# cocowy1/PPMStereo

Measured on AMD Instinct MI355X. Metric: disparity-px/s, higher is better.
Workload: dtype bf16

## Files before the change

### ppmstereo_amd/csrc/loop_ops.hip

```cpp
#include "common.h"

constexpr int DW_PX = 2;
template <int K>
__global__ __launch_bounds__(256) void dwconv_gelu_kernel(ppms_sp x, ppms_sp y, const float* __restrict__ w, const float* __restrict__ b,
                                                          int H, int W, int64_t rows, int groups) {
    __shared__ __attribute__((aligned(16))) float wl[K * K * 64];
    const int C = groups * 8;
    for (int i = threadIdx.x; i < K * K * C; i += 256) {
        const int c = i % C, tap = i / C;
        wl[tap * C + c] = w[c * K * K + tap];
    }
    __syncthreads();
    const int rpr = (W + DW_PX - 1) / DW_PX;
    const int64_t idx = (int64_t)blockIdx.x * 256 + threadIdx.x;
    if (idx >= rows * rpr * groups) return;
    const int c0 = (int)(idx % groups) * 8;
    const int64_t run = idx / groups;
    const int px0 = (int)(run % rpr) * DW_PX;
    const int64_t row = run / rpr;
    const int py = (int)(row % H);
    const int64_t pix0 = row * W + px0;
    const bf16_t* xh = (const bf16_t*)x.hi + c0;
    const bf16_t* xl = (const bf16_t*)x.lo + c0;
    float acc[DW_PX][8], x0[DW_PX][8];
    {
        const f32x4 b0 = *(const f32x4*)(b + c0), b1 = *(const f32x4*)(b + c0 + 4);
#pragma unroll
        for (int p = 0; p < DW_PX; ++p)
#pragma unroll
            for (int j = 0; j < 8; ++j) {
                acc[p][j] = j < 4 ? b0[j & 3] : b1[j & 3];
                x0[p][j] = 0.0f;
            }
    }
    constexpr int R = K / 2, NW = DW_PX + K - 1;
#pragma unroll
    for (int ky = 0; ky < K; ++ky) {
        const int yy = py + ky - R;
        if ((unsigned)yy >= (unsigned)H) continue;
        float win[NW][8];
#pragma unroll
        for (int i = 0; i < NW; ++i) {
            const int xx = px0 - R + i;
            bf16x8 h8 = {0, 0, 0, 0, 0, 0, 0, 0}, l8 = {0, 0, 0, 0, 0, 0, 0, 0};
            if ((unsigned)xx < (unsigned)W) {
                const int64_t q = pix0 + (int64_t)(ky - R) * W + (i - R);
                h8 = *(const bf16x8*)(xh + q * x.ld);
                l8 = *(const bf16x8*)(xl + q * x.ld);
            }
#pragma unroll
            for (int j = 0; j < 8; ++j) win[i][j] = join_bf16(h8[j], l8[j]);
        }
        if (ky == R) {
#pragma unroll
            for (int p = 0; p < DW_PX; ++p)
#pragma unroll
                for (int j = 0; j < 8; ++j) x0[p][j] = win[p + R][j];
        }
#pragma unroll
        for (int kx = 0; kx < K; ++kx) {
            const f32x4 w0 = *(const f32x4*)(wl + (ky * K + kx) * C + c0), w1 = *(const f32x4*)(wl + (ky * K + kx) * C + c0 + 4);
#pragma unroll
            for (int p = 0; p < DW_PX; ++p)
#pragma unroll
                for (int j = 0; j < 8; ++j) acc[p][j] += (j < 4 ? w0[j & 3] : w1[j & 3]) * win[p + kx][j];
        }
    }
#pragma unroll
    for (int p = 0; p < DW_PX; ++p) {
        if (px0 + p >= W) break;
        bf16x8 oh, ol;
#pragma unroll
        for (int j = 0; j < 8; ++j) {
            bf16_t hi, lo;
            split_bf16(gelu_erf(x0[p][j] + acc[p][j]), hi, lo);
            oh[j] = hi;
            ol[j] = lo;
        }
        *(bf16x8*)((bf16_t*)y.hi + (pix0 + p) * y.ld + c0) = oh;
        *(bf16x8*)((bf16_t*)y.lo + (pix0 + p) * y.ld + c0) = ol;
    }
}

extern "C" int ppms_dwconv_gelu(ppms_sp x, ppms_sp y, const float* w, const float* b, int k, int BT, int H, int W, void* stream) {
    PPMS_REQUIRE(k == 1 || k == 7, "dwconv_gelu: k=%d (only 1 and 7)", k);
    PPMS_REQUIRE(x.hi && x.lo && y.hi && y.lo && x.c == y.c && x.c > 0 && x.c <= 64 && x.c % 8 == 0 && x.ld % 8 == 0 && y.ld % 8 == 0,
                 "dwconv_gelu: views must have c <= 64 and c, ld multiples of 8");
    PPMS_REQUIRE((((uintptr_t)x.hi | (uintptr_t)x.lo | (uintptr_t)y.hi | (uintptr_t)y.lo) & 15) == 0,
                 "dwconv_gelu: the planes of x and y must be 16-byte aligned (a view starts at a multiple of 8 channels)");
    PPMS_REQUIRE(w != nullptr && b != nullptr && ((uintptr_t)b & 15) == 0, "dwconv_gelu: w and a 16-byte aligned bias expected");
    PPMS_REQUIRE(BT > 0 && H > 0 && W > 0, "dwconv_gelu: bad shape BT=%d H=%d W=%d", BT, H, W);
    const int64_t rows = (int64_t)BT * H;
    const int groups = x.c / 8;
    const dim3 grid(ceil_div(rows * ((W + DW_PX - 1) / DW_PX) * groups, 256));
    if (k == 1)
        hipLaunchKernelGGL(dwconv_gelu_kernel<1>, grid, dim3(256), 0, (hipStream_t)stream, x, y, w, b, H, W, rows, groups);
    else
        hipLaunchKernelGGL(dwconv_gelu_kernel<7>, grid, dim3(256), 0, (hipStream_t)stream, x, y, w, b, H, W, rows, groups);
    return ppms_check_launch("dwconv_gelu");
}

__global__ __launch_bounds__(256) void flow_patch7_kernel(const float* __restrict__ flow, ppms_sp patch, int H, int W, int64_t P) {
    const int64_t idx = (int64_t)blockIdx.x * 256 + threadIdx.x;
    if (idx >= P * 128) return;
    const int k = (int)(idx & 127);
    const int64_t pix = idx >> 7;
    float v = 0.0f;
    if (k < 98) {
        const int tap = k >> 1, c = k & 1;
        const int ky = tap / 7, kx = tap - ky * 7;
        const int px = (int)(pix % W), py = (int)((pix / W) % H);
        const int xx = px + kx - 3, yy = py + ky - 3;
        if ((unsigned)xx < (unsigned)W && (unsigned)yy < (unsigned)H) v = flow[(pix + (int64_t)(ky - 3) * W + (kx - 3)) * 2 + c];
    }
    bf16_t hi, lo;
    split_bf16(v, hi, lo);
    ((bf16_t*)patch.hi)[pix * patch.ld + k] = hi;
    ((bf16_t*)patch.lo)[pix * patch.ld + k] = lo;
}

extern "C" int ppms_flow_patch7(const float* flow_nhwc, ppms_sp patch, int BT, int H, int W, void* stream) {
    PPMS_REQUIRE(flow_nhwc && patch.hi && patch.lo && patch.ld >= 128, "flow_patch7: bad arguments");
    const int64_t P = (int64_t)BT * H * W;
    hipLaunchKernelGGL(flow_patch7_kernel, dim3(ceil_div(P * 128, 256)), dim3(256), 0, (hipStream_t)stream, flow_nhwc, patch, H, W, P);
    return ppms_check_launch("flow_patch7");
}

__global__ __launch_bounds__(256) void unc_tail_kernel(ppms_sp x, const float* __restrict__ w, float bias, float* __restrict__ unc,
                                                       float* __restrict__ partial, int HW, int nblk) {
    __shared__ float red[16];
    const int frame = blockIdx.y, blk = blockIdx.x;
    const int sub = threadIdx.x & 15, grp = threadIdx.x >> 4;
    float wv[8];
#pragma unroll
    for (int j = 0; j < 8; ++j) wv[j] = w[sub * 8 + j];
    bf16x8 h8[16], l8[16];
#pragma unroll
    for (int it = 0; it < 16; ++it) {
        const int pin = blk * 256 + it * 16 + grp;
        const int64_t pix = (int64_t)frame * HW + (pin < HW ? pin : HW - 1);
        h8[it] = gld<bf16x8>((const bf16_t*)x.hi + pix * x.ld + sub * 8);
        l8[it] = gld<bf16x8>((const bf16_t*)x.lo + pix * x.ld + sub * 8);
    }
    float local = 0.0f;
#pragma unroll
    for (int it = 0; it < 16; ++it) {
        const int pin = blk * 256 + it * 16 + grp;
        float s = 0.0f;
#pragma unroll
        for (int j = 0; j < 8; ++j) s += wv[j] * join_bf16(h8[it][j], l8[it][j]);
        s += __shfl_xor(s, 1);
        s += __shfl_xor(s, 2);
        s += __shfl_xor(s, 4);
        s += __shfl_xor(s, 8);
        if (pin < HW && sub == 0) {
            const float u = sigmoid_f(s + bias);
            unc[(int64_t)frame * HW + pin] = u;
            local += u;
        }
    }
    if (sub == 0) red[grp] = local;
    __syncthreads();
    if (threadIdx.x == 0) {
        float t = 0.0f;
        for (int i = 0; i < 16; ++i) t += red[i];
        partial[frame * nblk + blk] = t;
    }
}

extern "C" int ppms_unc_tail(ppms_sp x, const float* w, float bias, float* unc, float* partial, int BT, int HW, void* stream) {
    PPMS_REQUIRE(x.hi && x.lo && x.c == 128 && x.ld % 8 == 0, "unc_tail: expects a 128-channel SP view");
    const int nblk = ceil_div(HW, 256);
    hipLaunchKernelGGL(unc_tail_kernel, dim3(nblk, BT), dim3(256), 0, (hipStream_t)stream, x, w, bias, unc, partial, HW, nblk);
    return ppms_check_launch("unc_tail");
}

__global__ __launch_bounds__(256) void tap_gather_sum_kernel(const float* __restrict__ y, int y_ld, const float* __restrict__ bias,
                                                             float* __restrict__ out, int out_ld, float* __restrict__ accum, int accum_ld, int cout,
                                                             int kt, int kh, int kw, int T, int H, int W, int t_halo, int64_t total) {
    const int64_t idx = (int64_t)blockIdx.x * 256 + threadIdx.x;
    if (idx >= total) return;
    const int c = (int)(idx % cout);
    const int64_t pix = idx / cout;
    const int x = (int)(pix % W), yy = (int)((pix / W) % H), t = (int)(pix / ((int64_t)W * H));
    float acc = bias ? bias[c] : 0.0f;
    int tap = 0;
    for (int kz = 0; kz < kt; ++kz)
        for (int ky = 0; ky < kh; ++ky)
            for (int kx = 0; kx < kw; ++kx, ++tap) {
                const int tt = t + kz - kt / 2, y2 = yy + ky - kh / 2, x2 = x + kx - kw / 2;
                if ((unsigned)(tt + t_halo) < (unsigned)(T + 2 * t_halo) && (unsigned)y2 < (unsigned)H && (unsigned)x2 < (unsigned)W)
                    acc += y[(((int64_t)tt * H + y2) * W + x2) * y_ld + tap * cout + c];
            }
    out[pix * out_ld + c] = acc;
    if (accum != nullptr) accum[pix * accum_ld + c] += acc;
}
__global__ __launch_bounds__(256) void tap_gather_sum333_kernel(const float* __restrict__ y, int y_ld, const float* __restrict__ bias,
                                                                float* __restrict__ out, int out_ld, float* __restrict__ accum, int accum_ld, int cout,
                                                                int T, int H, int W, int t_halo, int64_t total) {
    const int64_t idx = (int64_t)blockIdx.x * 256 + threadIdx.x;
    if (idx >= total) return;
    const int c = (int)(idx % cout);
    const int64_t pix = idx / cout;
    const int x = (int)(pix % W), yy = (int)((pix / W) % H), t = (int)(pix / ((int64_t)W * H));
    float v[27];
#pragma unroll
    for (int tap = 0; tap < 27; ++tap) {
        const int kz = tap / 9, ky = (tap / 3) % 3, kx = tap % 3;
        const int tt = t + kz - 1, y2 = yy + ky - 1, x2 = x + kx - 1;
        const bool ok = (unsigned)(tt + t_halo) < (unsigned)(T + 2 * t_halo) && (unsigned)y2 < (unsigned)H && (unsigned)x2 < (unsigned)W;
        v[tap] = ok ? y[(((int64_t)tt * H + y2) * W + x2) * y_ld + tap * cout + c] : 0.0f;
    }
    float acc = bias ? bias[c] : 0.0f;
#pragma unroll
    for (int tap = 0; tap < 27; ++tap) {
        const int kz = tap / 9, ky = (tap / 3) % 3, kx = tap % 3;
        const int tt = t + kz - 1, y2 = yy + ky - 1, x2 = x + kx - 1;
        const bool ok = (unsigned)(tt + t_halo) < (unsigned)(T + 2 * t_halo) && (unsigned)y2 < (unsigned)H && (unsigned)x2 < (unsigned)W;
        if (ok) acc += v[tap];
    }
    out[pix * out_ld + c] = acc;
    if (accum != nullptr) accum[pix * accum_ld + c] += acc;
}
extern "C" int ppms_tap_gather_sum(const float* y, int y_ld, const float* bias, float* out, int out_ld, float* accum, int accum_ld, int cout, int kt,
                                   int kh, int kw, int T, int H, int W, int t_halo, void* stream) {
    PPMS_REQUIRE(y && out && cout > 0 && kt * kh * kw * cout <= y_ld && out_ld >= cout && t_halo >= 0, "tap_gather_sum: bad arguments");
    PPMS_REQUIRE(accum == nullptr || accum_ld >= cout, "tap_gather_sum: accum_ld=%d < cout=%d", accum_ld, cout);
    const int64_t total = (int64_t)T * H * W * cout;
    if (kt == 3 && kh == 3 && kw == 3)
        hipLaunchKernelGGL(tap_gather_sum333_kernel, dim3(ceil_div(total, 256)), dim3(256), 0, (hipStream_t)stream, y, y_ld, bias, out, out_ld, accum,
                           accum_ld, cout, T, H, W, t_halo, total);
    else
        hipLaunchKernelGGL(tap_gather_sum_kernel, dim3(ceil_div(total, 256)), dim3(256), 0, (hipStream_t)stream, y, y_ld, bias, out, out_ld, accum, accum_ld,
                           cout, kt, kh, kw, T, H, W, t_halo, total);
    return ppms_check_launch("tap_gather_sum");
}

__global__ __launch_bounds__(256) void flow_add_kernel(float* __restrict__ flow, const float* __restrict__ dflow, int dflow_ld, int64_t P) {
    const int64_t idx = (int64_t)blockIdx.x * 256 + threadIdx.x;
    if (idx >= P * 2) return;
    flow[idx] += dflow[(idx >> 1) * dflow_ld + (idx & 1)];
}
extern "C" int ppms_flow_add(float* flow_nhwc, const float* dflow, int dflow_ld, int64_t pixels, void* stream) {
    PPMS_REQUIRE(flow_nhwc && dflow && dflow_ld >= 2, "flow_add: bad arguments");
    hipLaunchKernelGGL(flow_add_kernel, dim3(ceil_div(pixels * 2, 256)), dim3(256), 0, (hipStream_t)stream, flow_nhwc, dflow, dflow_ld, pixels);
    return ppms_check_launch("flow_add");
}

__global__ __launch_bounds__(256) void convex_upsample_kernel(const float* __restrict__ flow, const float* __restrict__ mask, int mask_ld,
                                                              float* __restrict__ out, int H, int W, int64_t P) {
    const int64_t idx = (int64_t)blockIdx.x * 256 + threadIdx.x;
    if (idx >= P * 16) return;
    const int sub = (int)(idx & 15);
    const int64_t pix = idx >> 4;
    const int x = (int)(pix % W), y = (int)((pix / W) % H);
    const int64_t frame = pix / ((int64_t)H * W);
    const float* m = mask + pix * mask_ld + sub;
    float mv[9], mx = -INFINITY;
#pragma unroll
    for (int k = 0; k < 9; ++k) {
        mv[k] = m[16 * k];
        mx = fmaxf(mx, mv[k]);
    }
    float den = 0.0f;
#pragma unroll
    for (int k = 0; k < 9; ++k) {
        mv[k] = expf(mv[k] - mx);
        den += mv[k];
    }
    float o0 = 0.0f, o1 = 0.0f;
#pragma unroll
    for (int k = 0; k < 9; ++k) {
        const int yy = y + k / 3 - 1, xx = x + k % 3 - 1;
        if ((unsigned)yy < (unsigned)H && (unsigned)xx < (unsigned)W) {
            const int64_t q = pix + (int64_t)(k / 3 - 1) * W + (k % 3 - 1);
            const float wgt = mv[k] / den;
            o0 += wgt * (4.0f * flow[q * 2]);
            o1 += wgt * (4.0f * flow[q * 2 + 1]);
        }
    }
    const int i = sub >> 2, j = sub & 3;
    const int64_t OW = 4 * (int64_t)W, OHW = 16 * (int64_t)H * W;
    const int64_t o = (frame * 2) * OHW + (int64_t)(4 * y + i) * OW + 4 * x + j;
    out[o] = o0;
    out[o + OHW] = o1;
}
extern "C" int ppms_convex_upsample(const float* flow_nhwc, const float* mask, int mask_ld, float* out, int BT, int H, int W, void* stream) {
    PPMS_REQUIRE(flow_nhwc && mask && out && mask_ld >= 144, "convex_upsample: bad arguments");
    const int64_t P = (int64_t)BT * H * W;
    hipLaunchKernelGGL(convex_upsample_kernel, dim3(ceil_div(P * 16, 256)), dim3(256), 0, (hipStream_t)stream, flow_nhwc, mask, mask_ld,
                       out, H, W, P);
    return ppms_check_launch("convex_upsample");
}

__global__ __launch_bounds__(256) void convex_upsample3d_kernel(const float* __restrict__ flow, const float* __restrict__ mask, int mask_ld,
                                                                float* __restrict__ out, int T, int H, int W, int t_halo, int64_t P) {
    const int64_t idx = (int64_t)blockIdx.x * 256 + threadIdx.x;
    if (idx >= P * 16) return;
    const int sub = (int)(idx & 15);
    const int64_t pix = idx >> 4;
    const int x = (int)(pix % W), y = (int)((pix / W) % H);
    const int64_t frame = pix / ((int64_t)W * H);
    const float* mp = mask + pix * mask_ld + sub;
    float mv[27];
    float mx = mp[0];
#pragma unroll
    for (int k = 0; k < 27; ++k) {
        mv[k] = mp[16 * k];
        mx = fmaxf(mx, mv[k]);
    }
    float den = 0.0f;
#pragma unroll
    for (int k = 0; k < 27; ++k) {
        mv[k] = expf(mv[k] - mx);
        den += mv[k];
    }
    float o0 = 0.0f, o1 = 0.0f;
#pragma unroll
    for (int k = 0; k < 27; ++k) {
        const int dt = k / 9 - 1, dy = (k / 3) % 3 - 1, dx = k % 3 - 1;
        const int tt = (int)frame + dt, yy = y + dy, xx = x + dx;
        if ((unsigned)(tt + t_halo) < (unsigned)(T + 2 * t_halo) && (unsigned)yy < (unsigned)H && (unsigned)xx < (unsigned)W) {
            const int64_t q = pix + ((int64_t)dt * H + dy) * W + dx;
            const float wgt = mv[k] / den;
            o0 += wgt * (4.0f * flow[q * 2]);
            o1 += wgt * (4.0f * flow[q * 2 + 1]);
        }
    }
    const int i = sub >> 2, j = sub & 3;
    const int64_t OW = 4 * (int64_t)W, OHW = 16 * (int64_t)H * W;
    const int64_t o = (frame * 2) * OHW + (int64_t)(4 * y + i) * OW + 4 * x + j;
    out[o] = o0;
    out[o + OHW] = o1;
}
extern "C" int ppms_convex_upsample_3d(const float* flow_nhwc, const float* mask, int mask_ld, float* out, int T, int H, int W, int t_halo, void* stream) {
    PPMS_REQUIRE(flow_nhwc && mask && out && mask_ld >= 432 && T > 0 && H > 0 && W > 0 && t_halo >= 0, "convex_upsample_3d: bad arguments");
    const int64_t P = (int64_t)T * H * W;
    hipLaunchKernelGGL(convex_upsample3d_kernel, dim3(ceil_div(P * 16, 256)), dim3(256), 0, (hipStream_t)stream, flow_nhwc, mask, mask_ld,
                       out, T, H, W, t_halo, P);
    return ppms_check_launch("convex_upsample_3d");
}
```

Measured before the change: 23.59 million.

## Software-pipeline depthwise conv row loads and adapt per-thread tile to grid size

Rewrites the depthwise 7x7 conv+GELU kernel so input rows are prefetched several rows ahead into registers. Out-of-bounds taps are clamped rather than branched on, so loads stay unconditional. The kernel also overlaps the weight staging into shared memory with the first row loads, uses 32-bit offsets when the tensor fits, and joins hi/lo bf16 pairs with byte-permute ops. The launcher picks a smaller pixel/channel tile per thread when the grid would otherwise be too small, to keep the GPU occupied. The risk is higher register pressure from prefetch buffers and extra template instantiations.

```diff
diff --git a/ppmstereo_amd/csrc/loop_ops.hip b/ppmstereo_amd/csrc/loop_ops.hip
--- a/ppmstereo_amd/csrc/loop_ops.hip
+++ b/ppmstereo_amd/csrc/loop_ops.hip
@@ -1,85 +1,147 @@
 #include "common.h"
 
-constexpr int DW_PX = 2;
-template <int K>
+constexpr int dw_ahead(int NW, int CH) { return 176 / (NW * CH) < 1 ? 1 : 176 / (NW * CH); }
+constexpr int DW_MIN_THREADS = 65536;
+template <int PX, int CH> __device__ __forceinline__ void dw_pin(float (&a)[PX][CH]) {
+#pragma unroll
+    for (int p = 0; p < PX; ++p)
+#pragma unroll
+        for (int j = 0; j < CH; ++j) asm volatile("" : "+v"(a[p][j])::"memory");
+}
+template <int K, int PX, int CH, class OFS>
 __global__ __launch_bounds__(256) void dwconv_gelu_kernel(ppms_sp x, ppms_sp y, const float* __restrict__ w, const float* __restrict__ b,
                                                           int H, int W, int64_t rows, int groups) {
-    __shared__ __attribute__((aligned(16))) float wl[K * K * 64];
-    const int C = groups * 8;
-    for (int i = threadIdx.x; i < K * K * C; i += 256) {
-        const int c = i % C, tap = i / C;
-        wl[tap * C + c] = w[c * K * K + tap];
-    }
+    typedef bf16_t bfv __attribute__((ext_vector_type(CH)));
+    typedef float fv __attribute__((ext_vector_type(CH)));
+    constexpr int NT = 256;
+    __shared__ __attribute__((aligned(32))) float wl[K * K * 64];
+    constexpr int R = K / 2, NW = PX + K - 1, D = K < dw_ahead(NW, CH) ? K : dw_ahead(NW, CH);
+    const int C = groups * CH;
+    const int rpr = (W + PX - 1) / PX;
+    const OFS total = (OFS)rows * (OFS)rpr * (OFS)groups;
+    const OFS gid = (OFS)blockIdx.x * NT + threadIdx.x;
+    const bool live = gid < total;
+    const OFS idx = live ? gid : total - 1;
+    const OFS run = idx / (OFS)groups;
+    const int c0 = (int)(idx - run * (OFS)groups) * CH;
+    const OFS row = run / (OFS)rpr;
+    const int px0 = (int)(run - row * (OFS)rpr) * PX;
+    const int py = (int)(row % (OFS)H);
+    const int64_t pix0 = (int64_t)row * W + px0;
+    const char* xh = (const char*)x.hi;
+    const char* xl = (const char*)x.lo;
+    const OFS ldb = (OFS)x.ld * 2;
+    OFS col[NW];
+    bool cok[NW];
+#pragma unroll
+    for (int i = 0; i < NW; ++i) {
+        const int xx = px0 - R + i;
+        cok[i] = (unsigned)xx < (unsigned)W;
+        col[i] = (OFS)(xx < 0 ? 0 : (xx >= W ? W - 1 : xx)) * ldb + (OFS)(c0 * 2);
+    }
+    bfv rh[K][NW], rl[K][NW];
+    auto load_row = [&](int ky) __attribute__((always_inline)) {
+        const int yy = py + ky - R;
+        const OFS ro = (OFS)((row - py + (yy < 0 ? 0 : (yy >= H ? H - 1 : yy))) * W) * ldb;
+#pragma unroll
+        for (int i = 0; i < NW; ++i) {
+            rh[ky][i] = gld<bfv>(xh + (ro + col[i]));
+            rl[ky][i] = gld<bfv>(xl + (ro + col[i]));
+        }
+    };
+    float acc[PX][CH], x0[PX][CH];
+#pragma unroll
+    for (int j = 0; j < CH; ++j) acc[0][j] = gld<float>(b + c0 + j);
+#pragma unroll
+    for (int ky = 0; ky < D; ++ky) load_row(ky);
+#pragma unroll 4
+    for (int i = threadIdx.x; i < K * K * C; i += NT) {
+        const int c = i / (K * K), tap = i - c * (K * K);
+        wl[tap * C + c] = w[i];
+    }
+#pragma unroll
+    for (int p = 0; p < PX; ++p)
+#pragma unroll
+        for (int j = 0; j < CH; ++j) {
+            acc[p][j] = acc[0][j];
+            x0[p][j] = 0.0f;
+        }
     __syncthreads();
-    const int rpr = (W + DW_PX - 1) / DW_PX;
-    const int64_t idx = (int64_t)blockIdx.x * 256 + threadIdx.x;
-    if (idx >= rows * rpr * groups) return;
-    const int c0 = (int)(idx % groups) * 8;
-    const int64_t run = idx / groups;
-    const int px0 = (int)(run % rpr) * DW_PX;
-    const int64_t row = run / rpr;
-    const int py = (int)(row % H);
-    const int64_t pix0 = row * W + px0;
-    const bf16_t* xh = (const bf16_t*)x.hi + c0;
-    const bf16_t* xl = (const bf16_t*)x.lo + c0;
-    float acc[DW_PX][8], x0[DW_PX][8];
-    {
-        const f32x4 b0 = *(const f32x4*)(b + c0), b1 = *(const f32x4*)(b + c0 + 4);
-#pragma unroll
-        for (int p = 0; p < DW_PX; ++p)
-#pragma unroll
-            for (int j = 0; j < 8; ++j) {
-                acc[p][j] = j < 4 ? b0[j & 3] : b1[j & 3];
-                x0[p][j] = 0.0f;
+#pragma unroll
+    for (int ky = 0; ky < K; ++ky) {
+        const bool rok = K == 1 || (unsigned)(py + ky - R) < (unsigned)H;
+        float keep[PX][CH];
+#pragma unroll
+        for (int p = 0; p < PX; ++p)
+#pragma unroll
+            for (int j = 0; j < CH; ++j) keep[p][j] = acc[p][j];
+#pragma unroll
+        for (int i = 0; i < NW; ++i) {
+            unsigned hd[CH / 2], lw[CH / 2];
+            __builtin_memcpy(hd, &rh[ky][i], CH * 2);
+            __builtin_memcpy(lw, &rl[ky][i], CH * 2);
+            const unsigned m_odd = cok[i] ? 0xffff0000u : 0u, s_even = cok[i] ? 0x01000c0cu : 0x0c0c0c0cu;
+            float v[CH];
+#pragma unroll
+            for (int q = 0; q < CH / 2; ++q) {
+                v[2 * q] = __builtin_bit_cast(float, __builtin_amdgcn_perm(0u, hd[q], s_even)) + __builtin_bit_cast(float, __builtin_amdgcn_perm(0u, lw[q], s_even));
+                v[2 * q + 1] = __builtin_bit_cast(float, hd[q] & m_odd) + __builtin_bit_cast(float, lw[q] & m_odd);
             }
-    }
-    constexpr int R = K / 2, NW = DW_PX + K - 1;
-#pragma unroll
-    for (int ky = 0; ky < K; ++ky) {
-        const int yy = py + ky - R;
-        if ((unsigned)yy >= (unsigned)H) continue;
-        float win[NW][8];
-#pragma unroll
-        for (int i = 0; i < NW; ++i) {
-            const int xx = px0 - R + i;
-            bf16x8 h8 = {0, 0, 0, 0, 0, 0, 0, 0}, l8 = {0, 0, 0, 0, 0, 0, 0, 0};
-            if ((unsigned)xx < (unsigned)W) {
-                const int64_t q = pix0 + (int64_t)(ky - R) * W + (i - R);
-                h8 = *(const bf16x8*)(xh + q * x.ld);
-                l8 = *(const bf16x8*)(xl + q * x.ld);
+            if (ky == R && i >= R && i < R + PX) {
+#pragma unroll
+                for (int j = 0; j < CH; ++j) x0[i - R][j] = v[j];
             }
 #pragma unroll
-            for (int j = 0; j < 8; ++j) win[i][j] = join_bf16(h8[j], l8[j]);
-        }
-        if (ky == R) {
-#pragma unroll
-            for (int p = 0; p < DW_PX; ++p)
-#pragma unroll
-                for (int j = 0; j < 8; ++j) x0[p][j] = win[p + R][j];
-        }
-#pragma unroll
-        for (int kx = 0; kx < K; ++kx) {
-            const f32x4 w0 = *(const f32x4*)(wl + (ky * K + kx) * C + c0), w1 = *(const f32x4*)(wl + (ky * K + kx) * C + c0 + 4);
-#pragma unroll
-            for (int p = 0; p < DW_PX; ++p)
-#pragma unroll
-                for (int j = 0; j < 8; ++j) acc[p][j] += (j < 4 ? w0[j & 3] : w1[j & 3]) * win[p + kx][j];
-        }
-    }
-#pragma unroll
-    for (int p = 0; p < DW_PX; ++p) {
-        if (px0 + p >= W) break;
-        bf16x8 oh, ol;
-#pragma unroll
-        for (int j = 0; j < 8; ++j) {
+            for (int p = 0; p < PX; ++p) {
+                const int kx = i - p;
+                if (kx < 0 || kx >= K) continue;
+                const fv wv = *(const fv*)(wl + (ky * K + kx) * C + c0);
+#pragma unroll
+                for (int j = 0; j < CH; ++j) acc[p][j] += wv[j] * v[j];
+            }
+        }
+#pragma unroll
+        for (int p = 0; p < PX; ++p)
+#pragma unroll
+            for (int j = 0; j < CH; ++j) acc[p][j] = rok ? acc[p][j] : keep[p][j];
+        dw_pin(acc);
+        if (ky + D < K) load_row(ky + D);
+    }
+#pragma unroll
+    for (int p = 0; p < PX; ++p) {
+        if (!live || px0 + p >= W) break;
+        bfv oh, ol;
+#pragma unroll
+        for (int j = 0; j < CH; ++j) {
             bf16_t hi, lo;
             split_bf16(gelu_erf(x0[p][j] + acc[p][j]), hi, lo);
             oh[j] = hi;
             ol[j] = lo;
         }
-        *(bf16x8*)((bf16_t*)y.hi + (pix0 + p) * y.ld + c0) = oh;
-        *(bf16x8*)((bf16_t*)y.lo + (pix0 + p) * y.ld + c0) = ol;
-    }
+        gst<bfv>((bf16_t*)y.hi + (pix0 + p) * y.ld + c0, oh);
+        gst<bfv>((bf16_t*)y.lo + (pix0 + p) * y.ld + c0, ol);
+    }
+}
+
+template <int PX, int CH> static int64_t dwconv_threads(int64_t rows, int W, int c) { return rows * ((W + PX - 1) / PX) * (c / CH); }
+template <int K, int PX, int CH>
+static void dwconv_launch(ppms_sp x, ppms_sp y, const float* w, const float* b, int H, int W, int64_t rows, void* stream) {
+    const dim3 grid(ceil_div(dwconv_threads<PX, CH>(rows, W, x.c), 256));
+    if ((uint64_t)rows * W * x.ld * 2 <= 0xffffffffull)
+        hipLaunchKernelGGL((dwconv_gelu_kernel<K, PX, CH, uint32_t>), grid, dim3(256), 0, (hipStream_t)stream, x, y, w, b, H, W, rows, x.c / CH);
+    else
+        hipLaunchKernelGGL((dwconv_gelu_kernel<K, PX, CH, uint64_t>), grid, dim3(256), 0, (hipStream_t)stream, x, y, w, b, H, W, rows, x.c / CH);
+}
+template <int K>
+static void dwconv_shape(ppms_sp x, ppms_sp y, const float* w, const float* b, int H, int W, int64_t rows, void* stream) {
+    if (dwconv_threads<2, 8>(rows, W, x.c) >= DW_MIN_THREADS)
+        dwconv_launch<K, 2, 8>(x, y, w, b, H, W, rows, stream);
+    else if (dwconv_threads<1, 8>(rows, W, x.c) >= DW_MIN_THREADS)
+        dwconv_launch<K, 1, 8>(x, y, w, b, H, W, rows, stream);
+    else if (dwconv_threads<1, 4>(rows, W, x.c) >= DW_MIN_THREADS)
+        dwconv_launch<K, 1, 4>(x, y, w, b, H, W, rows, stream);
+    else
+        dwconv_launch<K, 1, 2>(x, y, w, b, H, W, rows, stream);
 }
 
 extern "C" int ppms_dwconv_gelu(ppms_sp x, ppms_sp y, const float* w, const float* b, int k, int BT, int H, int W, void* stream) {
@@ -91,12 +153,10 @@
     PPMS_REQUIRE(w != nullptr && b != nullptr && ((uintptr_t)b & 15) == 0, "dwconv_gelu: w and a 16-byte aligned bias expected");
     PPMS_REQUIRE(BT > 0 && H > 0 && W > 0, "dwconv_gelu: bad shape BT=%d H=%d W=%d", BT, H, W);
     const int64_t rows = (int64_t)BT * H;
-    const int groups = x.c / 8;
-    const dim3 grid(ceil_div(rows * ((W + DW_PX - 1) / DW_PX) * groups, 256));
     if (k == 1)
-        hipLaunchKernelGGL(dwconv_gelu_kernel<1>, grid, dim3(256), 0, (hipStream_t)stream, x, y, w, b, H, W, rows, groups);
+        dwconv_shape<1>(x, y, w, b, H, W, rows, stream);
     else
-        hipLaunchKernelGGL(dwconv_gelu_kernel<7>, grid, dim3(256), 0, (hipStream_t)stream, x, y, w, b, H, W, rows, groups);
+        dwconv_shape<7>(x, y, w, b, H, W, rows, stream);
     return ppms_check_launch("dwconv_gelu");
 }
 
```

New measurement: 23.55 million. Within noise of the previous version (-0.2%).
